# NtagkasAlex/phase_guided_terrain_traversal

Measured on AMD Instinct MI355X. Metric: env-steps/sec at 4096 envs (Go2, level4 hfield), 1/2/4/8 MI355X, higher is better.
Workload: dtype f32

## Files before the change

include/pgtt_train.h:

```cpp
#ifndef PGTT_TRAIN_H_
#define PGTT_TRAIN_H_
#include "pgtt.h"
#ifdef __cplusplus
extern "C" {
#endif
int pgtt_ppo_policy_loss(const float* out_Bx2A, const float* u_BxA, const float* logp_old_B, const float* adv_B,
                         const float* eps_BxA, int B, int A, float clip_eps, float entropy_cost,
                         float* partial_2xceilB64, float* loss_3, float* grad_Bx2A, void* stream);
int pgtt_ppo_linear_backward(const float* x_KxM, const float* dy_KxN, int K, int M, int N, int S,
                             float* partial_Sx_NM_plus_N, float* dw_NxM, float* db_N, void* stream);

typedef struct PgttPolicyActArgs {
  const float* obs;
  const float* priv;
  const float* mean;
  const float* std;
  const float* w[4];
  const float* b[4];
  const float* eps;
  float* act;
  float* head;
  float* store_obs;
  float* store_priv;
  float* store_u;
  float* store_logp;
  const int64_t* counters;
  uint64_t seed;
  int64_t env_id_offset;
  int32_t num_envs, obs_dim, priv_dim;
  int32_t deterministic;
  int32_t store_rows;
} PgttPolicyActArgs;
int pgtt_policy_act(const PgttPolicyActArgs* args, void* stream);
int pgtt_policy_packed_floats(int in_dim, int out_dim);

typedef struct PgttRolloutRecordArgs {
  const float* reward;
  const float* done;
  const int32_t* ep_steps;
  const float* up_z;
  const float* ep_metrics;
  float* store_rew;
  float* store_done;
  float* store_trunc;
  int64_t* counters;
  float* episode_sums;
  float reward_scaling;
  int32_t num_envs, episode_length;
  int32_t store_rows;
} PgttRolloutRecordArgs;
int pgtt_rollout_record(const PgttRolloutRecordArgs* args, void* stream);
int pgtt_sizeof_policy_act_args(void);
int pgtt_sizeof_rollout_record_args(void);
#ifdef __cplusplus
}
#endif
#endif
```

phase_guided_terrain_traversal_amd/acting.py:

```python
from __future__ import annotations

import ctypes as C
from typing import Dict, List, Optional, Sequence, Tuple

import torch
import torch.nn.functional as F

from . import abi, native

_f, _i32, _p = C.c_float, C.c_int32, C.c_void_p


class PgttPolicyActArgs(C.Structure):
    _fields_ = [("obs", _p), ("priv", _p), ("mean", _p), ("std", _p), ("w", _p * 4), ("b", _p * 4), ("eps", _p), ("act", _p), ("head", _p),
                ("store_obs", _p), ("store_priv", _p), ("store_u", _p), ("store_logp", _p), ("counters", _p), ("seed", C.c_uint64),
                ("env_id_offset", C.c_int64), ("num_envs", _i32), ("obs_dim", _i32), ("priv_dim", _i32), ("deterministic", _i32), ("store_rows", _i32)]


class PgttRolloutRecordArgs(C.Structure):
    _fields_ = [("reward", _p), ("done", _p), ("ep_steps", _p), ("up_z", _p), ("ep_metrics", _p), ("store_rew", _p), ("store_done", _p),
                ("store_trunc", _p), ("counters", _p), ("episode_sums", _p), ("reward_scaling", _f),
                ("num_envs", _i32), ("episode_length", _i32), ("store_rows", _i32)]


HIDDEN = (512, 256, 128)


def _lib():
    L = native.lib()
    if not getattr(L, "_acting_ready", False):
        L.pgtt_policy_act.argtypes = [C.POINTER(PgttPolicyActArgs), _p]
        L.pgtt_rollout_record.argtypes = [C.POINTER(PgttRolloutRecordArgs), _p]
        L.pgtt_policy_packed_floats.argtypes = [C.c_int, C.c_int]
        assert L.pgtt_sizeof_policy_act_args() == C.sizeof(PgttPolicyActArgs) and L.pgtt_sizeof_rollout_record_args() == C.sizeof(PgttRolloutRecordArgs)
        L._acting_ready = True
    return L


def pack_linear(w: torch.Tensor, b: torch.Tensor) -> Tuple[torch.Tensor, torch.Tensor]:
    n, k = w.shape
    npad, kpad = -(-n // 16) * 16, -(-k // 16) * 16
    wp = F.pad(w.detach().float(), (0, kpad - k, 0, npad - n))
    packed = wp.view(npad // 16, 16, kpad // 16, 4, 4).permute(0, 2, 3, 1, 4).contiguous().reshape(-1)
    return packed, F.pad(b.detach().float(), (0, npad - n)).contiguous()


class FusedActor:

    def __init__(self, env, T: int, seed: int = 0, reward_scaling: float = 1.0, episode_sums: Optional[torch.Tensor] = None,
                 obs: Optional[torch.Tensor] = None):
        if env.device.type != "cuda":
            raise native.PgttError("FusedActor needs a Joystick on a ROCm device; there is no CPU path")
        self.env, self.T = env, int(T)
        self._L = _lib()
        dev, n = env.device, env.num_envs
        od, pd = env.observation_size["state"], env.observation_size["privileged_state"]
        self.od, self.pd = od, pd
        z = lambda *sh: torch.zeros(*sh, device=dev)
        self.storage: Dict[str, torch.Tensor] = {"obs": z(T, n, od), "priv": z(T, n, pd), "u": z(T, n, abi.NU), "logp": z(T, n), "rew": z(T, n),
                                                  "done": z(T, n), "trunc": z(T, n)}
        self.action = z(n, abi.NU)
        self.counters = torch.zeros(2, dtype=torch.int64, device=dev)
        self.episode_sums = z(abi.NMETRIC + 3) if episode_sums is None else episode_sums
        assert self.episode_sums.numel() == abi.NMETRIC + 3 and self.episode_sums.is_contiguous()
        self.mean, self.std = z(od), torch.ones(od, device=dev)
        dims = (od,) + HIDDEN + (2 * abi.NU,)
        self._w = [z(self._L.pgtt_policy_packed_floats(dims[l], dims[l + 1])) for l in range(4)]
        self._b = [z(-(-dims[l + 1] // 16) * 16) for l in range(4)]
        self._dims = dims
        a = PgttPolicyActArgs()
        self.obs = env.buffers["obs_state"] if obs is None else obs
        if not (self.obs.dtype == torch.float32 and self.obs.is_contiguous() and tuple(self.obs.shape) == (n, od) and self.obs.device == env.buffers["obs_state"].device):
            raise ValueError(f"FusedActor: `obs` must be {n} x {od} contiguous float32 values on {dev}")
        a.obs, a.priv = self.obs.data_ptr(), env.buffers["obs_priv"].data_ptr()
        a.mean, a.std = self.mean.data_ptr(), self.std.data_ptr()
        for l in range(4):
            a.w[l], a.b[l] = self._w[l].data_ptr(), self._b[l].data_ptr()
        a.eps, a.head, a.act = None, None, self.action.data_ptr()
        S = self.storage
        a.store_obs, a.store_priv, a.store_u, a.store_logp = S["obs"].data_ptr(), S["priv"].data_ptr(), S["u"].data_ptr(), S["logp"].data_ptr()
        a.counters, a.seed, a.env_id_offset = self.counters.data_ptr(), int(seed) & 0xFFFFFFFFFFFFFFFF, int(env.env_id_offset)
        a.num_envs, a.obs_dim, a.priv_dim, a.deterministic, a.store_rows = n, od, pd, 0, self.T
        self._act_args = a
        r = PgttRolloutRecordArgs()
        r.reward, r.done = env.buffers["reward"].data_ptr(), env.buffers["done"].data_ptr()
        r.ep_steps = env.buffers["istate"][abi.I_EP_STEPS].data_ptr()
        r.up_z = env.buffers["frame"][abi.F_UPVECTOR + 2].data_ptr()
        r.ep_metrics = env.buffers["ep_metrics"].data_ptr()
        r.store_rew, r.store_done, r.store_trunc = S["rew"].data_ptr(), S["done"].data_ptr(), S["trunc"].data_ptr()
        r.counters, r.episode_sums = self.counters.data_ptr(), self.episode_sums.data_ptr()
        r.reward_scaling, r.num_envs, r.episode_length, r.store_rows = float(reward_scaling), n, int(env.config["episode_length"]), self.T
        self._rec_args = r

    def _stream(self) -> int:
        return torch.cuda.current_stream(self.env.device).cuda_stream

    @torch.no_grad()
    def load(self, layers: Sequence[Tuple[torch.Tensor, torch.Tensor]], mean: torch.Tensor, std: torch.Tensor) -> None:
        assert len(layers) == 4
        for l, (w, b) in enumerate(layers):
            assert tuple(w.shape) == (self._dims[l + 1], self._dims[l]), (l, tuple(w.shape), self._dims)
            pw, pb = pack_linear(w.to(self.mean.device), b.to(self.mean.device))
            self._w[l].copy_(pw); self._b[l].copy_(pb)
        self.mean.copy_(mean); self.std.copy_(std)

    def load_sequential(self, seq: torch.nn.Sequential, mean: torch.Tensor, std: torch.Tensor) -> None:
        lins = [m for m in seq if isinstance(m, torch.nn.Linear)]
        self.load([(m.weight, m.bias) for m in lins], mean, std)

    def act(self, deterministic: bool = False, eps: Optional[torch.Tensor] = None, head: Optional[torch.Tensor] = None, store: bool = True) -> torch.Tensor:
        a = self._act_args
        a.deterministic = int(deterministic)
        a.eps = None if eps is None else eps.data_ptr()
        a.head = None if head is None else head.data_ptr()
        if eps is not None:
            assert eps.is_contiguous() and eps.dtype == torch.float32 and tuple(eps.shape) == (self.env.num_envs, abi.NU)
        S = self.storage
        a.store_obs, a.store_priv, a.store_u, a.store_logp = ((S["obs"].data_ptr(), S["priv"].data_ptr(), S["u"].data_ptr(), S["logp"].data_ptr())
                                                              if store else (None, None, None, None))
        native.check(self._L.pgtt_policy_act(C.byref(a), self._stream()))
        return self.action

    def record(self) -> None:
        native.check(self._L.pgtt_rollout_record(C.byref(self._rec_args), self._stream()))

    def step(self) -> None:
        self.act()
        if getattr(self.env, "curriculum", None) is not None:
            self.env.step(self.action, curriculum=False)
            self.record()
            self.env.curriculum_step()
            return
        self.env.step(self.action)
        self.record()

    def rewind(self) -> None:
        self.counters[0].zero_()
```

phase_guided_terrain_traversal_amd/csrc/pgtt_policy.hip:

```cpp
#include <hip/hip_runtime.h>
#include <math.h>
#include "../../include/pgtt_train.h"

namespace {

typedef float f32x4 __attribute__((ext_vector_type(4)));

constexpr int kEnvs = 16;
constexpr int kH1 = 512, kH2 = 256, kH3 = 128;
constexpr int kOut = 24, kOutPad = 32;
constexpr int kA = 12;
constexpr int kMaxObsPad = 224;

__device__ inline float softplus_t(float x) { return x > 20.f ? x : log1pf(expf(x)); }
__device__ inline float silu(float x) { return x / (1.0f + expf(-x)); }

__device__ inline void philox4x32_10(unsigned k0, unsigned k1, unsigned& c0, unsigned& c1, unsigned& c2, unsigned& c3) {
#pragma unroll
  for (int r = 0; r < 10; r++) {
    const unsigned h0 = __umulhi(0xD2511F53u, c0), l0 = 0xD2511F53u * c0;
    const unsigned h1 = __umulhi(0xCD9E8D57u, c2), l1 = 0xCD9E8D57u * c2;
    const unsigned n0 = h1 ^ c1 ^ k0, n2 = h0 ^ c3 ^ k1;
    c0 = n0; c1 = l1; c2 = n2; c3 = l0;
    k0 += 0x9E3779B9u; k1 += 0xBB67AE85u;
  }
}

template <int NT, int KB, int DEPTH>
__device__ inline void layer_tiles(const float4* __restrict__ Wp, const float* __restrict__ X, int KS, int tile0, f32x4 (&acc)[NT]) {
  const int lane = threadIdx.x & 63;
  const float* xrow = X + (lane & 15) * KS + 4 * (lane >> 4);
  const float4* wl = Wp + (long)tile0 * KB * 64 + lane;
  float4 a[DEPTH][NT];
#pragma unroll
  for (int d = 0; d < DEPTH; d++)
#pragma unroll
    for (int t = 0; t < NT; t++) if (d < KB) a[d][t] = wl[(t * KB + d) * 64];
#pragma unroll
  for (int t = 0; t < NT; t++) acc[t] = f32x4{0.f, 0.f, 0.f, 0.f};
  float4 bq[2];
  bq[0] = *reinterpret_cast<const float4*>(xrow);
#pragma unroll
  for (int kb = 0; kb < KB; kb++) {
    const float4 b = bq[kb & 1];
    if (kb + 1 < KB) bq[(kb + 1) & 1] = *reinterpret_cast<const float4*>(xrow + 16 * (kb + 1));
    float4 cur[NT];
#pragma unroll
    for (int t = 0; t < NT; t++) cur[t] = a[kb % DEPTH][t];
    if (kb + DEPTH < KB) {
#pragma unroll
      for (int t = 0; t < NT; t++) a[kb % DEPTH][t] = wl[(t * KB + kb + DEPTH) * 64];
    }
    __builtin_amdgcn_sched_barrier(0);
#pragma unroll
    for (int t = 0; t < NT; t++) acc[t] = __builtin_amdgcn_mfma_f32_16x16x4f32(cur[t].x, b.x, acc[t], 0, 0, 0);
#pragma unroll
    for (int t = 0; t < NT; t++) acc[t] = __builtin_amdgcn_mfma_f32_16x16x4f32(cur[t].y, b.y, acc[t], 0, 0, 0);
#pragma unroll
    for (int t = 0; t < NT; t++) acc[t] = __builtin_amdgcn_mfma_f32_16x16x4f32(cur[t].z, b.z, acc[t], 0, 0, 0);
#pragma unroll
    for (int t = 0; t < NT; t++) acc[t] = __builtin_amdgcn_mfma_f32_16x16x4f32(cur[t].w, b.w, acc[t], 0, 0, 0);
    __builtin_amdgcn_sched_barrier(0);
  }
}

template <int NT, bool ACT>
__device__ inline void store_tiles(const f32x4 (&acc)[NT], const float* __restrict__ bias, int tile0, float* __restrict__ Xout, int KS) {
  const int lane = threadIdx.x & 63, i = lane & 15, g = lane >> 4;
#pragma unroll
  for (int t = 0; t < NT; t++) {
    const int n = 16 * (tile0 + t) + 4 * g;
    const float4 bv = *reinterpret_cast<const float4*>(bias + n);
    float4 v = make_float4(acc[t][0] + bv.x, acc[t][1] + bv.y, acc[t][2] + bv.z, acc[t][3] + bv.w);
    if (ACT) { v.x = silu(v.x); v.y = silu(v.y); v.z = silu(v.z); v.w = silu(v.w); }
    *reinterpret_cast<float4*>(Xout + i * KS + n) = v;
  }
}

constexpr int kWaves = 8;
constexpr int kThreads = 64 * kWaves;

__global__ __launch_bounds__(kThreads) void policy_act_kernel(PgttPolicyActArgs a) {
  __shared__ __attribute__((aligned(16))) float bufA[kEnvs * (kH1 + 4)];
  __shared__ __attribute__((aligned(16))) float bufB[kEnvs * (kH2 + 4)];
  __shared__ float sh_lp[kEnvs * kA];
  const int tid = threadIdx.x, wave = tid >> 6;
  const int N = a.num_envs, od = a.obs_dim, kp0 = (od + 15) & ~15, ks0 = kp0 + 4, kb0n = kp0 >> 4;
  const long e0 = (long)blockIdx.x * kEnvs;
  const long t_row = a.counters ? a.counters[0] : 0;
  const bool row_ok = t_row >= 0 && t_row < a.store_rows;
  const float4* W0 = reinterpret_cast<const float4*>(a.w[0]);
  {
    constexpr int kObsTrips = kMaxObsPad / 32;
    constexpr int kPrivTrips = (kEnvs * kMaxObsPad + kThreads - 1) / kThreads;
    const int env = tid >> 5, k0 = tid & 31;
    const long e = e0 + env;
    const bool copy_priv = a.store_priv && a.priv && row_ok;
    const int pd = a.priv_dim;
    const long pbase = e0 * pd, plim = (long)N * pd;
    float o[kObsTrips], mu[kObsTrips], sd[kObsTrips], pv[kPrivTrips];
#pragma unroll
    for (int j = 0; j < kObsTrips; j++) {
      const int k = k0 + 32 * j;
      const bool in = k < od && e < N;
      o[j] = in ? a.obs[e * od + k] : 0.f; mu[j] = in ? a.mean[k] : 0.f; sd[j] = in ? a.std[k] : 1.f;
    }
#pragma unroll
    for (int j = 0; j < kPrivTrips; j++) {
      const int idx = tid + kThreads * j;
      pv[j] = (copy_priv && idx < kEnvs * pd && pbase + idx < plim) ? a.priv[pbase + idx] : 0.f;
    }
#pragma unroll
    for (int j = 0; j < kObsTrips; j++) {
      const int k = k0 + 32 * j;
      if (k < kp0) bufB[env * ks0 + k] = (k < od && e < N) ? (o[j] - mu[j]) / sd[j] : 0.f;
      if (a.store_obs && row_ok && k < od && e < N) a.store_obs[(t_row * N + e) * od + k] = o[j];
    }
#pragma unroll
    for (int j = 0; j < kPrivTrips; j++) {
      const int idx = tid + kThreads * j;
      if (copy_priv && idx < kEnvs * pd && pbase + idx < plim) a.store_priv[t_row * N * pd + pbase + idx] = pv[j];
    }
  }
  __syncthreads();
  {
    f32x4 acc[4];
    if (kb0n == 11) layer_tiles<4, 11, 4>(W0, bufB, ks0, 4 * wave, acc);
    else if (kb0n == 14) layer_tiles<4, 14, 4>(W0, bufB, ks0, 4 * wave, acc);
    else {
      const int lane = tid & 63;
      const float* xrow = bufB + (lane & 15) * ks0 + 4 * (lane >> 4);
#pragma unroll
      for (int t = 0; t < 4; t++) acc[t] = f32x4{0.f, 0.f, 0.f, 0.f};
      for (int kb = 0; kb < kb0n; kb++) {
        const float4 b = *reinterpret_cast<const float4*>(xrow + 16 * kb);
#pragma unroll
        for (int t = 0; t < 4; t++) {
          const float4 w = W0[((long)(4 * wave + t) * kb0n + kb) * 64 + lane];
          acc[t] = __builtin_amdgcn_mfma_f32_16x16x4f32(w.x, b.x, acc[t], 0, 0, 0); acc[t] = __builtin_amdgcn_mfma_f32_16x16x4f32(w.y, b.y, acc[t], 0, 0, 0);
          acc[t] = __builtin_amdgcn_mfma_f32_16x16x4f32(w.z, b.z, acc[t], 0, 0, 0); acc[t] = __builtin_amdgcn_mfma_f32_16x16x4f32(w.w, b.w, acc[t], 0, 0, 0);
        }
      }
    }
    store_tiles<4, true>(acc, a.b[0], 4 * wave, bufA, kH1 + 4);
  }
  __syncthreads();
  {
    f32x4 acc[2];
    layer_tiles<2, kH1 / 16, 8>(reinterpret_cast<const float4*>(a.w[1]), bufA, kH1 + 4, 2 * wave, acc);
    store_tiles<2, true>(acc, a.b[1], 2 * wave, bufB, kH2 + 4);
  }
  __syncthreads();
  {
    f32x4 acc[1];
    layer_tiles<1, kH2 / 16, 8>(reinterpret_cast<const float4*>(a.w[2]), bufB, kH2 + 4, wave, acc);
    store_tiles<1, true>(acc, a.b[2], wave, bufA, kH3 + 4);
  }
  __syncthreads();
  if (wave < 2) {
    f32x4 acc[1];
    layer_tiles<1, kH3 / 16, 8>(reinterpret_cast<const float4*>(a.w[3]), bufA, kH3 + 4, wave, acc);
    store_tiles<1, false>(acc, a.b[3], wave, bufB, kOutPad + 4);
  }
  __syncthreads();
  if (tid < kEnvs * kA) {
    const int env = tid / kA, j = tid - env * kA;
    const long e = e0 + env;
    const float loc = bufB[env * (kOutPad + 4) + j], raw = bufB[env * (kOutPad + 4) + kA + j];
    const float sc = softplus_t(raw) + 1e-3f;
    float eps;
    if (a.eps) eps = e < N ? a.eps[e * kA + j] : 0.f;
    else {
      const unsigned long long draw = a.counters ? (unsigned long long)a.counters[1] : 0ull;
      unsigned c0 = (unsigned)(a.env_id_offset + e), c1 = (unsigned)draw, c2 = (unsigned)(draw >> 32) ^ 0x50475454u, c3 = (unsigned)(j >> 1);
      philox4x32_10((unsigned)a.seed, (unsigned)(a.seed >> 32), c0, c1, c2, c3);
      const float u1 = ((float)(c0 >> 8) + 0.5f) * (1.0f / 16777216.0f), u2 = (float)(c1 >> 8) * (1.0f / 16777216.0f);
      const float r = sqrtf(-2.0f * logf(u1));
      float sn, cs; sincosf(6.28318530717958648f * u2, &sn, &cs);
      eps = (j & 1) ? r * sn : r * cs;
    }
    const float u = a.deterministic ? loc : loc + sc * eps;
    const float z = (u - loc) / sc;
    const float kHalfLog2Pi = 0.91893853320467274f, kLog2 = 0.69314718055994531f;
    sh_lp[tid] = -0.5f * z * z - logf(sc) - kHalfLog2Pi - 2.0f * (kLog2 - u - softplus_t(-2.0f * u));
    if (e < N) {
      const float th = tanhf(u);
      a.act[e * kA + j] = th;
      if (a.store_u && row_ok) a.store_u[(t_row * N + e) * kA + j] = u;
      if (a.head) { a.head[e * kOut + j] = loc; a.head[e * kOut + kA + j] = raw; }
    }
  }
  __syncthreads();
  if (tid < kEnvs && e0 + tid < N && a.store_logp && row_ok) {
    float lp = 0.f;
#pragma unroll
    for (int j = 0; j < kA; j++) lp += sh_lp[tid * kA + j];
    a.store_logp[t_row * N + e0 + tid] = lp;
  }
}

constexpr int kRecSums = PGTT_NMETRIC + 3;
constexpr int kRecThreads = 1024;

__global__ __launch_bounds__(kRecThreads) void rollout_record_kernel(PgttRolloutRecordArgs a) {
  __shared__ float sh[kRecSums][kRecThreads / 64];
  const int tid = threadIdx.x, lane = tid & 63, wave = tid >> 6;
  const int N = a.num_envs;
  const long t_row = a.counters[0];
  const long draws = a.counters[1];
  const bool row_ok = t_row >= 0 && t_row < a.store_rows;
  float sums[kRecSums];
#pragma unroll
  for (int k = 0; k < kRecSums; k++) sums[k] = 0.f;
  bool any = false;
  for (int e = tid; e < N; e += kRecThreads) {
    const float done = a.done[e], rew = a.reward[e];
    const bool fallen = a.up_z[e] < 0.f;
    const bool trunc = (a.ep_steps[e] >= a.episode_length) && !fallen;
    if (row_ok) {
      a.store_rew[t_row * N + e] = rew * a.reward_scaling;
      a.store_done[t_row * N + e] = done;
      a.store_trunc[t_row * N + e] = trunc ? 1.f : 0.f;
    }
    if (done != 0.f) {
      any = true;
#pragma unroll
      for (int k = 0; k < PGTT_NMETRIC + 2; k++) sums[k] += a.ep_metrics[(long)k * N + e] * done;
      sums[PGTT_NMETRIC + 2] += done;
    }
  }
  if (__syncthreads_or(any ? 1 : 0)) {
#pragma unroll
    for (int k = 0; k < kRecSums; k++) {
      float v = sums[k];
#pragma unroll
      for (int o = 32; o > 0; o >>= 1) v += __shfl_xor(v, o);
      if (lane == 0) sh[k][wave] = v;
    }
    __syncthreads();
    if (tid < kRecSums) {
      float v = 0.f;
#pragma unroll
      for (int w = 0; w < kRecThreads / 64; w++) v += sh[tid][w];
      a.episode_sums[tid] += v;
    }
  }
  if (tid == 0) { a.counters[0] = t_row + 1; a.counters[1] = draws + 1; }
}

}

extern "C" int pgtt_policy_act(const PgttPolicyActArgs* args, void* stream) {
  if (!args || !args->obs || !args->mean || !args->std || !args->act || args->num_envs <= 0) return PGTT_E_ARG;
  for (int l = 0; l < 4; l++) if (!args->w[l] || !args->b[l]) return PGTT_E_ARG;
  if (args->obs_dim <= 0 || ((args->obs_dim + 15) & ~15) > kMaxObsPad) return PGTT_E_ARG;
  if (args->store_priv && (!args->priv || args->priv_dim <= 0 || args->priv_dim > kMaxObsPad)) return PGTT_E_ARG;
  if ((args->store_obs || args->store_priv || args->store_u || args->store_logp) && args->store_rows <= 0) return PGTT_E_ARG;
  hipLaunchKernelGGL(policy_act_kernel, dim3((args->num_envs + kEnvs - 1) / kEnvs), dim3(kThreads), 0, (hipStream_t)stream, *args);
  return hipGetLastError() == hipSuccess ? PGTT_OK : PGTT_E_HIP;
}

extern "C" int pgtt_rollout_record(const PgttRolloutRecordArgs* args, void* stream) {
  if (!args || !args->reward || !args->done || !args->ep_steps || !args->up_z || !args->ep_metrics || !args->store_rew || !args->store_done ||
      !args->store_trunc || !args->counters || !args->episode_sums || args->num_envs <= 0 || args->store_rows <= 0) return PGTT_E_ARG;
  hipLaunchKernelGGL(rollout_record_kernel, dim3(1), dim3(kRecThreads), 0, (hipStream_t)stream, *args);
  return hipGetLastError() == hipSuccess ? PGTT_OK : PGTT_E_HIP;
}

extern "C" int pgtt_policy_packed_floats(int in_dim, int out_dim) { return ((out_dim + 15) & ~15) * ((in_dim + 15) & ~15); }
extern "C" int pgtt_sizeof_policy_act_args(void) { return (int)sizeof(PgttPolicyActArgs); }
extern "C" int pgtt_sizeof_rollout_record_args(void) { return (int)sizeof(PgttRolloutRecordArgs); }
```

phase_guided_terrain_traversal_amd/native.py:

```python
from __future__ import annotations

import ctypes as C
import os
from typing import Optional

from . import abi

_HERE = os.path.dirname(os.path.abspath(__file__))
LIB_PATH = os.environ.get("PGTT_LIB", os.path.join(_HERE, "libpgtt.so"))
_LIB: Optional[C.CDLL] = None

EXPORTS = ["pgtt_create", "pgtt_destroy", "pgtt_set_terrain", "pgtt_bind", "pgtt_reset", "pgtt_step",
           "pgtt_physics", "pgtt_observe", "pgtt_scan", "pgtt_push", "pgtt_curriculum", "pgtt_curriculum_check", "pgtt_set_curriculum", "pgtt_set_curriculum_deferred", "pgtt_sizeof_curriculum", "pgtt_interval_reduce", "pgtt_set_test_overrides", "pgtt_enable_timing", "pgtt_last_kernel_ms", "pgtt_kernel_ms_mean",
           "pgtt_obs_dims", "pgtt_sizeof_model", "pgtt_sizeof_config", "pgtt_sizeof_buffers", "pgtt_version", "pgtt_build_info", "pgtt_last_error"]
TRAIN_EXPORTS = ["pgtt_ppo_policy_loss", "pgtt_ppo_linear_backward", "pgtt_policy_act", "pgtt_policy_packed_floats", "pgtt_rollout_record",
                 "pgtt_sizeof_policy_act_args", "pgtt_sizeof_rollout_record_args"]


class PgttError(RuntimeError):
    pass


def source_sha256() -> str:
    from . import srchash
    return srchash.source_sha256()


def build_info(path: Optional[str] = None) -> dict:
    if path or _LIB is None:
        import torch
        L = C.CDLL(path or LIB_PATH)
    else:
        L = _LIB
    L.pgtt_build_info.restype = C.c_char_p
    return dict(kv.split("=", 1) for kv in L.pgtt_build_info().decode().split(";"))


def library_sha256(path: Optional[str] = None) -> str:
    import hashlib
    with open(path or LIB_PATH, "rb") as fh:
        return hashlib.sha256(fh.read()).hexdigest()


def lib() -> C.CDLL:
    global _LIB
    if _LIB is None:
        if not os.path.exists(LIB_PATH):
            raise PgttError(f"{LIB_PATH} not found: build it with `python -c 'import __graft_entry__ as g; g.build()'` "
                            "(hipcc --offload-arch=gfx950); there is no CPU fallback")
        import torch
        L = C.CDLL(LIB_PATH)
        L.pgtt_last_error.restype = C.c_char_p
        L.pgtt_version.restype = C.c_char_p
        L.pgtt_create.argtypes = [C.POINTER(abi.PgttConfig), C.POINTER(abi.PgttModel), C.c_int, C.c_int, C.POINTER(C.c_void_p)]
        L.pgtt_destroy.argtypes = [C.c_void_p]
        L.pgtt_set_terrain.argtypes = [C.c_void_p, C.c_void_p, C.c_int, C.c_int]
        L.pgtt_bind.argtypes = [C.c_void_p, C.POINTER(abi.PgttBuffers)]
        L.pgtt_reset.argtypes = [C.c_void_p, C.c_uint64, C.c_int64, C.c_void_p, C.c_void_p]
        for fn in ("pgtt_step", "pgtt_physics", "pgtt_observe"):
            getattr(L, fn).argtypes = [C.c_void_p, C.c_void_p, C.c_void_p]
        L.pgtt_scan.argtypes = [C.c_void_p, C.c_float, C.c_void_p]
        L.pgtt_push.argtypes = [C.c_void_p, C.c_void_p]
        L.pgtt_curriculum.argtypes = [C.c_void_p, C.c_void_p]
        L.pgtt_set_curriculum_deferred.argtypes = [C.c_void_p, C.c_int]
        L.pgtt_set_curriculum.argtypes = [C.c_void_p, C.POINTER(abi.PgttCurriculum)]
        L.pgtt_curriculum_check.argtypes = [C.POINTER(abi.PgttConfig), C.POINTER(abi.PgttCurriculum)]
        L.pgtt_interval_reduce.argtypes = [C.c_void_p, C.c_void_p, C.c_float, C.c_int, C.c_void_p]
        L.pgtt_enable_timing.argtypes = [C.c_void_p, C.c_int]
        L.pgtt_set_test_overrides.argtypes = [C.c_void_p, C.c_float, C.c_int]
        L.pgtt_last_kernel_ms.argtypes = [C.c_void_p, C.POINTER(C.c_float), C.POINTER(C.c_float)]
        assert L.pgtt_sizeof_model() == C.sizeof(abi.PgttModel)
        assert L.pgtt_sizeof_config() == C.sizeof(abi.PgttConfig)
        assert L.pgtt_sizeof_buffers() == C.sizeof(abi.PgttBuffers)
        assert L.pgtt_sizeof_curriculum() == C.sizeof(abi.PgttCurriculum)
        _LIB = L
    return _LIB


def check(rc: int) -> None:
    if rc != 0:
        raise PgttError(f"libpgtt error {rc}: {lib().pgtt_last_error().decode()}")
```

Before: 22.68 million.

## Split policy MLP into tiled layer kernels with global workspace for wider parallelism

Replaces the single fused per-block policy kernel with three launches: a layer-1 kernel and a layer-2 kernel, each tiled over 64 envs by neuron-column groups across a 2D grid, writing activations to a global workspace, then a tail kernel that reads layer-2 output and finishes the head and sampling. The aim is to spread the wide hidden layers over more blocks so each block re-reads fewer weights and utilisation improves at 4096 envs. The layer-2 kernel double-buffers chunks of layer-1 activations through LDS. The cost is extra launches and a global-memory round trip for the activations. Separately, the rollout record kernel batches four env loads per thread to raise memory-level parallelism.

```diff
diff --git a/include/pgtt_train.h b/include/pgtt_train.h
--- a/include/pgtt_train.h
+++ b/include/pgtt_train.h
@@ -30,9 +30,11 @@
   int32_t num_envs, obs_dim, priv_dim;
   int32_t deterministic;
   int32_t store_rows;
+  float* workspace;
 } PgttPolicyActArgs;
 int pgtt_policy_act(const PgttPolicyActArgs* args, void* stream);
 int pgtt_policy_packed_floats(int in_dim, int out_dim);
+int pgtt_policy_workspace_floats(int num_envs);
 
 typedef struct PgttRolloutRecordArgs {
   const float* reward;
diff --git a/phase_guided_terrain_traversal_amd/acting.py b/phase_guided_terrain_traversal_amd/acting.py
--- a/phase_guided_terrain_traversal_amd/acting.py
+++ b/phase_guided_terrain_traversal_amd/acting.py
@@ -14,7 +14,8 @@
 class PgttPolicyActArgs(C.Structure):
     _fields_ = [("obs", _p), ("priv", _p), ("mean", _p), ("std", _p), ("w", _p * 4), ("b", _p * 4), ("eps", _p), ("act", _p), ("head", _p),
                 ("store_obs", _p), ("store_priv", _p), ("store_u", _p), ("store_logp", _p), ("counters", _p), ("seed", C.c_uint64),
-                ("env_id_offset", C.c_int64), ("num_envs", _i32), ("obs_dim", _i32), ("priv_dim", _i32), ("deterministic", _i32), ("store_rows", _i32)]
+                ("env_id_offset", C.c_int64), ("num_envs", _i32), ("obs_dim", _i32), ("priv_dim", _i32), ("deterministic", _i32), ("store_rows", _i32),
+                ("workspace", _p)]
 
 
 class PgttRolloutRecordArgs(C.Structure):
@@ -32,6 +33,7 @@
         L.pgtt_policy_act.argtypes = [C.POINTER(PgttPolicyActArgs), _p]
         L.pgtt_rollout_record.argtypes = [C.POINTER(PgttRolloutRecordArgs), _p]
         L.pgtt_policy_packed_floats.argtypes = [C.c_int, C.c_int]
+        L.pgtt_policy_workspace_floats.argtypes = [C.c_int]
         assert L.pgtt_sizeof_policy_act_args() == C.sizeof(PgttPolicyActArgs) and L.pgtt_sizeof_rollout_record_args() == C.sizeof(PgttRolloutRecordArgs)
         L._acting_ready = True
     return L
@@ -81,6 +83,11 @@
         a.store_obs, a.store_priv, a.store_u, a.store_logp = S["obs"].data_ptr(), S["priv"].data_ptr(), S["u"].data_ptr(), S["logp"].data_ptr()
         a.counters, a.seed, a.env_id_offset = self.counters.data_ptr(), int(seed) & 0xFFFFFFFFFFFFFFFF, int(env.env_id_offset)
         a.num_envs, a.obs_dim, a.priv_dim, a.deterministic, a.store_rows = n, od, pd, 0, self.T
+        nws = self._L.pgtt_policy_workspace_floats(n)
+        if nws <= 0:
+            raise native.PgttError(f"pgtt_policy_workspace_floats({n}) = {nws}")
+        self._workspace = z(nws)
+        a.workspace = self._workspace.data_ptr()
         self._act_args = a
         r = PgttRolloutRecordArgs()
         r.reward, r.done = env.buffers["reward"].data_ptr(), env.buffers["done"].data_ptr()
diff --git a/phase_guided_terrain_traversal_amd/csrc/pgtt_policy.hip b/phase_guided_terrain_traversal_amd/csrc/pgtt_policy.hip
--- a/phase_guided_terrain_traversal_amd/csrc/pgtt_policy.hip
+++ b/phase_guided_terrain_traversal_amd/csrc/pgtt_policy.hip
@@ -1,5 +1,7 @@
 #include <hip/hip_runtime.h>
+#include <limits.h>
 #include <math.h>
+#include <stdint.h>
 #include "../../include/pgtt_train.h"
 
 namespace {
@@ -80,8 +82,9 @@
 constexpr int kWaves = 8;
 constexpr int kThreads = 64 * kWaves;
 
+template <bool TAIL>
 __global__ __launch_bounds__(kThreads) void policy_act_kernel(PgttPolicyActArgs a) {
-  __shared__ __attribute__((aligned(16))) float bufA[kEnvs * (kH1 + 4)];
+  __shared__ __attribute__((aligned(16))) float bufA[kEnvs * ((TAIL ? kH3 : kH1) + 4)];
   __shared__ __attribute__((aligned(16))) float bufB[kEnvs * (kH2 + 4)];
   __shared__ float sh_lp[kEnvs * kA];
   const int tid = threadIdx.x, wave = tid >> 6;
@@ -89,6 +92,15 @@
   const long e0 = (long)blockIdx.x * kEnvs;
   const long t_row = a.counters ? a.counters[0] : 0;
   const bool row_ok = t_row >= 0 && t_row < a.store_rows;
+  if constexpr (TAIL) {
+    const float* H2 = a.workspace + (long)N * kH1;
+#pragma unroll
+    for (int j = 0; j < kEnvs * kH2 / 4 / kThreads; j++) {
+      const int idx = tid + kThreads * j, env = idx / (kH2 / 4), c4 = idx % (kH2 / 4);
+      const float4 v = e0 + env < N ? *reinterpret_cast<const float4*>(H2 + (e0 + env) * kH2 + 4 * c4) : make_float4(0.f, 0.f, 0.f, 0.f);
+      *reinterpret_cast<float4*>(bufB + env * (kH2 + 4) + 4 * c4) = v;
+    }
+  } else {
   const float4* W0 = reinterpret_cast<const float4*>(a.w[0]);
   {
     constexpr int kObsTrips = kMaxObsPad / 32;
@@ -149,6 +161,7 @@
     f32x4 acc[2];
     layer_tiles<2, kH1 / 16, 8>(reinterpret_cast<const float4*>(a.w[1]), bufA, kH1 + 4, 2 * wave, acc);
     store_tiles<2, true>(acc, a.b[1], 2 * wave, bufB, kH2 + 4);
+  }
   }
   __syncthreads();
   {
@@ -199,8 +212,183 @@
   }
 }
 
+constexpr int kTileEnvs = 64;
+constexpr int kTileWaves = 4;
+constexpr int kTileThreads = 64 * kTileWaves;
+constexpr int kEnvTiles = kTileEnvs / kEnvs;
+constexpr int kChunkKB = 8;
+constexpr int kChunkStride = 16 * kChunkKB + 4;
+
+struct NoStage {
+  __device__ inline void fetch(int) {}
+  __device__ inline void commit(int) {}
+};
+
+struct H1Stage {
+  const float* src;
+  float* lds;
+  int rows;
+  float4 r[kTileEnvs * kChunkKB * 4 / kTileThreads];
+  __device__ inline void fetch(int c) {
+#pragma unroll
+    for (int j = 0; j < kTileEnvs * kChunkKB * 4 / kTileThreads; j++) {
+      const int idx = threadIdx.x + kTileThreads * j, row = idx / (4 * kChunkKB), c4 = idx % (4 * kChunkKB);
+      r[j] = row < rows ? *reinterpret_cast<const float4*>(src + (long)row * kH1 + 16 * kChunkKB * c + 4 * c4) : make_float4(0.f, 0.f, 0.f, 0.f);
+    }
+  }
+  __device__ inline void commit(int c) {
+#pragma unroll
+    for (int j = 0; j < kTileEnvs * kChunkKB * 4 / kTileThreads; j++) {
+      const int idx = threadIdx.x + kTileThreads * j, row = idx / (4 * kChunkKB), c4 = idx % (4 * kChunkKB);
+      *reinterpret_cast<float4*>(lds + (c & 1) * kTileEnvs * kChunkStride + row * kChunkStride + 4 * c4) = r[j];
+    }
+  }
+};
+
+template <int KB, int CH, int DEPTH, class Stage>
+__device__ inline void env_tiles(const float4* __restrict__ wl, const float* X, int KS, int bufStride, Stage& stage, f32x4 (&acc)[kEnvTiles]) {
+  const int lane = threadIdx.x & 63;
+  const float* xrow = X + (lane & 15) * KS + 4 * (lane >> 4);
+  float4 a[DEPTH];
+#pragma unroll
+  for (int d = 0; d < DEPTH; d++) if (d < KB) a[d] = wl[d * 64];
+#pragma unroll
+  for (int t = 0; t < kEnvTiles; t++) acc[t] = f32x4{0.f, 0.f, 0.f, 0.f};
+  float4 bq[2][kEnvTiles];
+#pragma unroll
+  for (int kb = 0; kb < KB; kb++) {
+    const int c = kb / CH, j = kb % CH;
+    const float* xc = xrow + (c & 1) * bufStride + 16 * j;
+    if (j == 0) {
+      if ((c + 1) * CH < KB) stage.fetch(c + 1);
+#pragma unroll
+      for (int t = 0; t < kEnvTiles; t++) bq[kb & 1][t] = *reinterpret_cast<const float4*>(xc + t * kEnvs * KS);
+    }
+    if (j + 1 < CH && kb + 1 < KB) {
+#pragma unroll
+      for (int t = 0; t < kEnvTiles; t++) bq[(kb + 1) & 1][t] = *reinterpret_cast<const float4*>(xc + 16 + t * kEnvs * KS);
+    }
+    const float4 cur = a[kb % DEPTH];
+    if (kb + DEPTH < KB) a[kb % DEPTH] = wl[(kb + DEPTH) * 64];
+    __builtin_amdgcn_sched_barrier(0);
+#pragma unroll
+    for (int t = 0; t < kEnvTiles; t++) acc[t] = __builtin_amdgcn_mfma_f32_16x16x4f32(cur.x, bq[kb & 1][t].x, acc[t], 0, 0, 0);
+#pragma unroll
+    for (int t = 0; t < kEnvTiles; t++) acc[t] = __builtin_amdgcn_mfma_f32_16x16x4f32(cur.y, bq[kb & 1][t].y, acc[t], 0, 0, 0);
+#pragma unroll
+    for (int t = 0; t < kEnvTiles; t++) acc[t] = __builtin_amdgcn_mfma_f32_16x16x4f32(cur.z, bq[kb & 1][t].z, acc[t], 0, 0, 0);
+#pragma unroll
+    for (int t = 0; t < kEnvTiles; t++) acc[t] = __builtin_amdgcn_mfma_f32_16x16x4f32(cur.w, bq[kb & 1][t].w, acc[t], 0, 0, 0);
+    __builtin_amdgcn_sched_barrier(0);
+    if (j == CH - 1 && kb + 1 < KB) { stage.commit(c + 1); __syncthreads(); }
+  }
+}
+
+__device__ inline void store_env_tiles(const f32x4 (&acc)[kEnvTiles], const float* __restrict__ bias, int tile, float* __restrict__ H, int LD, long e0, int N) {
+  const int lane = threadIdx.x & 63, i = lane & 15, g = lane >> 4;
+  const int n = 16 * tile + 4 * g;
+  const float4 bv = *reinterpret_cast<const float4*>(bias + n);
+#pragma unroll
+  for (int t = 0; t < kEnvTiles; t++) {
+    const long e = e0 + kEnvs * t + i;
+    const float4 v = make_float4(silu(acc[t][0] + bv.x), silu(acc[t][1] + bv.y), silu(acc[t][2] + bv.z), silu(acc[t][3] + bv.w));
+    if (e < N) *reinterpret_cast<float4*>(H + e * LD + n) = v;
+  }
+}
+
+__global__ __launch_bounds__(kTileThreads) void policy_l1_kernel(PgttPolicyActArgs a) {
+  __shared__ __attribute__((aligned(16))) float xs[kTileEnvs * (kMaxObsPad + 4)];
+  const int tid = threadIdx.x, wave = tid >> 6, lane = tid & 63;
+  const int N = a.num_envs, od = a.obs_dim, kp0 = (od + 15) & ~15, ks0 = kp0 + 4, kb0n = kp0 >> 4;
+  const long e0 = (long)blockIdx.x * kTileEnvs;
+  const int col = blockIdx.y;
+  const long t_row = a.counters ? a.counters[0] : 0;
+  const bool row_ok = t_row >= 0 && t_row < a.store_rows;
+  {
+    constexpr int kObsTrips = kMaxObsPad / 32;
+    constexpr int kRounds = kTileEnvs / (kTileThreads / 32);
+    constexpr int kPrivTrips = (kTileEnvs * kMaxObsPad + kRounds * kTileThreads - 1) / (kRounds * kTileThreads);
+    const int h = tid >> 5, k0 = tid & 31;
+    const bool copy_priv = a.store_priv && a.priv && row_ok;
+    const int pd = a.priv_dim;
+    const long pbase = e0 * pd, plim = (long)N * pd;
+    float mu[kObsTrips], sd[kObsTrips], pv[kPrivTrips];
+#pragma unroll
+    for (int j = 0; j < kObsTrips; j++) {
+      const int k = k0 + 32 * j;
+      mu[j] = k < od ? a.mean[k] : 0.f; sd[j] = k < od ? a.std[k] : 1.f;
+    }
+#pragma unroll
+    for (int j = 0; j < kPrivTrips; j++) {
+      const int idx = tid + kTileThreads * (col + kRounds * j);
+      pv[j] = (copy_priv && idx < kTileEnvs * pd && pbase + idx < plim) ? a.priv[pbase + idx] : 0.f;
+    }
+#pragma unroll 2
+    for (int r = 0; r < kRounds; r++) {
+      const int env = (kTileThreads / 32) * r + h;
+      const long e = e0 + env;
+      float o[kObsTrips];
+#pragma unroll
+      for (int j = 0; j < kObsTrips; j++) {
+        const int k = k0 + 32 * j;
+        o[j] = (k < od && e < N) ? a.obs[e * od + k] : 0.f;
+      }
+#pragma unroll
+      for (int j = 0; j < kObsTrips; j++) {
+        const int k = k0 + 32 * j;
+        if (k < kp0) xs[env * ks0 + k] = (k < od && e < N) ? (o[j] - mu[j]) / sd[j] : 0.f;
+        if (a.store_obs && row_ok && r == col && k < od && e < N) a.store_obs[(t_row * N + e) * od + k] = o[j];
+      }
+    }
+#pragma unroll
+    for (int j = 0; j < kPrivTrips; j++) {
+      const int idx = tid + kTileThreads * (col + kRounds * j);
+      if (copy_priv && idx < kTileEnvs * pd && pbase + idx < plim) a.store_priv[t_row * N * pd + pbase + idx] = pv[j];
+    }
+    static_assert(kRounds == kH1 / (16 * kTileWaves), "one observation round per neuron column");
+  }
+  __syncthreads();
+  const int tile = kTileWaves * col + wave;
+  const float4* wl = reinterpret_cast<const float4*>(a.w[0]) + (long)tile * kb0n * 64 + lane;
+  f32x4 acc[kEnvTiles];
+  NoStage none;
+  if (kb0n == 11) env_tiles<11, 11, 4>(wl, xs, ks0, 0, none, acc);
+  else if (kb0n == 14) env_tiles<14, 14, 4>(wl, xs, ks0, 0, none, acc);
+  else {
+    const float* xrow = xs + (lane & 15) * ks0 + 4 * (lane >> 4);
+#pragma unroll
+    for (int t = 0; t < kEnvTiles; t++) acc[t] = f32x4{0.f, 0.f, 0.f, 0.f};
+    for (int kb = 0; kb < kb0n; kb++) {
+      const float4 w = wl[kb * 64];
+#pragma unroll
+      for (int t = 0; t < kEnvTiles; t++) {
+        const float4 b = *reinterpret_cast<const float4*>(xrow + t * kEnvs * ks0 + 16 * kb);
+        acc[t] = __builtin_amdgcn_mfma_f32_16x16x4f32(w.x, b.x, acc[t], 0, 0, 0); acc[t] = __builtin_amdgcn_mfma_f32_16x16x4f32(w.y, b.y, acc[t], 0, 0, 0);
+        acc[t] = __builtin_amdgcn_mfma_f32_16x16x4f32(w.z, b.z, acc[t], 0, 0, 0); acc[t] = __builtin_amdgcn_mfma_f32_16x16x4f32(w.w, b.w, acc[t], 0, 0, 0);
+      }
+    }
+  }
+  store_env_tiles(acc, a.b[0], tile, a.workspace, kH1, e0, N);
+}
+
+__global__ __launch_bounds__(kTileThreads) void policy_l2_kernel(PgttPolicyActArgs a) {
+  __shared__ __attribute__((aligned(16))) float xs[2 * kTileEnvs * kChunkStride];
+  const int wave = threadIdx.x >> 6, lane = threadIdx.x & 63;
+  const int N = a.num_envs;
+  const long e0 = (long)blockIdx.x * kTileEnvs;
+  const int tile = kTileWaves * blockIdx.y + wave;
+  H1Stage stage;
+  stage.src = a.workspace + e0 * kH1; stage.lds = xs; stage.rows = (int)(N - e0 < kTileEnvs ? N - e0 : kTileEnvs);
+  stage.fetch(0); stage.commit(0);
+  __syncthreads();
+  f32x4 acc[kEnvTiles];
+  env_tiles<kH1 / 16, kChunkKB, 4>(reinterpret_cast<const float4*>(a.w[1]) + (long)tile * (kH1 / 16) * 64 + lane, xs, kChunkStride, kTileEnvs * kChunkStride, stage, acc);
+  store_env_tiles(acc, a.b[1], tile, a.workspace + (long)N * kH1, kH2, e0, N);
+}
+
 constexpr int kRecSums = PGTT_NMETRIC + 3;
 constexpr int kRecThreads = 1024;
+constexpr int kRecBatch = 4;
 
 __global__ __launch_bounds__(kRecThreads) void rollout_record_kernel(PgttRolloutRecordArgs a) {
   __shared__ float sh[kRecSums][kRecThreads / 64];
@@ -213,20 +401,30 @@
 #pragma unroll
   for (int k = 0; k < kRecSums; k++) sums[k] = 0.f;
   bool any = false;
-  for (int e = tid; e < N; e += kRecThreads) {
-    const float done = a.done[e], rew = a.reward[e];
-    const bool fallen = a.up_z[e] < 0.f;
-    const bool trunc = (a.ep_steps[e] >= a.episode_length) && !fallen;
-    if (row_ok) {
-      a.store_rew[t_row * N + e] = rew * a.reward_scaling;
-      a.store_done[t_row * N + e] = done;
-      a.store_trunc[t_row * N + e] = trunc ? 1.f : 0.f;
-    }
-    if (done != 0.f) {
-      any = true;
-#pragma unroll
-      for (int k = 0; k < PGTT_NMETRIC + 2; k++) sums[k] += a.ep_metrics[(long)k * N + e] * done;
-      sums[PGTT_NMETRIC + 2] += done;
+  for (int base = tid; base < N; base += kRecThreads * kRecBatch) {
+    float done[kRecBatch], rew[kRecBatch], upz[kRecBatch];
+    int steps[kRecBatch];
+#pragma unroll
+    for (int j = 0; j < kRecBatch; j++) {
+      const int e = min(base + kRecThreads * j, N - 1);
+      done[j] = a.done[e]; rew[j] = a.reward[e]; upz[j] = a.up_z[e]; steps[j] = a.ep_steps[e];
+    }
+#pragma unroll
+    for (int j = 0; j < kRecBatch; j++) {
+      const int e = base + kRecThreads * j;
+      if (e >= N) continue;
+      const bool trunc = (steps[j] >= a.episode_length) && !(upz[j] < 0.f);
+      if (row_ok) {
+        a.store_rew[t_row * N + e] = rew[j] * a.reward_scaling;
+        a.store_done[t_row * N + e] = done[j];
+        a.store_trunc[t_row * N + e] = trunc ? 1.f : 0.f;
+      }
+      if (done[j] != 0.f) {
+        any = true;
+#pragma unroll
+        for (int k = 0; k < PGTT_NMETRIC + 2; k++) sums[k] += a.ep_metrics[(long)k * N + e] * done[j];
+        sums[PGTT_NMETRIC + 2] += done[j];
+      }
     }
   }
   if (__syncthreads_or(any ? 1 : 0)) {
@@ -248,6 +446,11 @@
   if (tid == 0) { a.counters[0] = t_row + 1; a.counters[1] = draws + 1; }
 }
 
+}
+
+extern "C" int pgtt_policy_workspace_floats(int num_envs) {
+  if (num_envs <= 0 || num_envs > INT_MAX / (kH1 + kH2)) return PGTT_E_ARG;
+  return num_envs * (kH1 + kH2);
 }
 
 extern "C" int pgtt_policy_act(const PgttPolicyActArgs* args, void* stream) {
@@ -256,7 +459,18 @@
   if (args->obs_dim <= 0 || ((args->obs_dim + 15) & ~15) > kMaxObsPad) return PGTT_E_ARG;
   if (args->store_priv && (!args->priv || args->priv_dim <= 0 || args->priv_dim > kMaxObsPad)) return PGTT_E_ARG;
   if ((args->store_obs || args->store_priv || args->store_u || args->store_logp) && args->store_rows <= 0) return PGTT_E_ARG;
-  hipLaunchKernelGGL(policy_act_kernel, dim3((args->num_envs + kEnvs - 1) / kEnvs), dim3(kThreads), 0, (hipStream_t)stream, *args);
+  const dim3 grid((args->num_envs + kEnvs - 1) / kEnvs);
+  if (!args->workspace) {
+    hipLaunchKernelGGL(policy_act_kernel<false>, grid, dim3(kThreads), 0, (hipStream_t)stream, *args);
+    return hipGetLastError() == hipSuccess ? PGTT_OK : PGTT_E_HIP;
+  }
+  if (((uintptr_t)args->workspace & 15) || pgtt_policy_workspace_floats(args->num_envs) < 0) return PGTT_E_ARG;
+  const unsigned tiles = (args->num_envs + kTileEnvs - 1) / kTileEnvs;
+  hipLaunchKernelGGL(policy_l1_kernel, dim3(tiles, kH1 / (16 * kTileWaves)), dim3(kTileThreads), 0, (hipStream_t)stream, *args);
+  if (hipGetLastError() != hipSuccess) return PGTT_E_HIP;
+  hipLaunchKernelGGL(policy_l2_kernel, dim3(tiles, kH2 / (16 * kTileWaves)), dim3(kTileThreads), 0, (hipStream_t)stream, *args);
+  if (hipGetLastError() != hipSuccess) return PGTT_E_HIP;
+  hipLaunchKernelGGL(policy_act_kernel<true>, grid, dim3(kThreads), 0, (hipStream_t)stream, *args);
   return hipGetLastError() == hipSuccess ? PGTT_OK : PGTT_E_HIP;
 }
 
diff --git a/phase_guided_terrain_traversal_amd/native.py b/phase_guided_terrain_traversal_amd/native.py
--- a/phase_guided_terrain_traversal_amd/native.py
+++ b/phase_guided_terrain_traversal_amd/native.py
@@ -14,7 +14,7 @@
            "pgtt_physics", "pgtt_observe", "pgtt_scan", "pgtt_push", "pgtt_curriculum", "pgtt_curriculum_check", "pgtt_set_curriculum", "pgtt_set_curriculum_deferred", "pgtt_sizeof_curriculum", "pgtt_interval_reduce", "pgtt_set_test_overrides", "pgtt_enable_timing", "pgtt_last_kernel_ms", "pgtt_kernel_ms_mean",
            "pgtt_obs_dims", "pgtt_sizeof_model", "pgtt_sizeof_config", "pgtt_sizeof_buffers", "pgtt_version", "pgtt_build_info", "pgtt_last_error"]
 TRAIN_EXPORTS = ["pgtt_ppo_policy_loss", "pgtt_ppo_linear_backward", "pgtt_policy_act", "pgtt_policy_packed_floats", "pgtt_rollout_record",
-                 "pgtt_sizeof_policy_act_args", "pgtt_sizeof_rollout_record_args"]
+                 "pgtt_sizeof_policy_act_args", "pgtt_sizeof_rollout_record_args", "pgtt_policy_workspace_floats"]
 
 
 class PgttError(RuntimeError):
```

Result: no change. 22.68 million (median of 4 runs) (+0.0%).
